# fperezgamonal/flownet2-tf

Hardware: AMD Instinct MI355X
Metric: forward pairs/sec at 512x384 (FlowNet2) (higher is better)
Workload: dtype f16x2 (split fp16 hi+lo operands, 3 fp16 MFMAs per product, fp32 accumulate); 1 GPU; FlowNet2 forward, batch=4 synthetic 512x384 pairs per GPU, seeded synthetic weights; pairs_per_gpu=4, parallelism=dp1 (no collective)

## Files before the change

flownet2-tf_amd/csrc/conv.hip:

```cpp
#include "conv_common.h"
#include <cstdlib>

namespace fn2 {

template <typename T, typename OutT, int TC, int WC, int WP>
__global__ void __launch_bounds__(256) conv_igemm_kernel(const ConvArgs p) {
  constexpr int CH = 16 / (int)sizeof(T);
  constexpr int BC = WC * TC * 16;
  constexpr int BP = WP * 64;
  constexpr int NT = 256;
  static_assert(WC * WP == 4, "4 waves per block");
  constexpr int NPR = BP / 64;
  constexpr int NWR = (BC * 4 + NT - 1) / NT;
  constexpr int WSWZ_BIT = (TC == 4) ? 5 : (TC == 2) ? 4 : 3;
  __shared__ uint4 lds[2][(BC + BP) * 4];

  const int tid = threadIdx.x, lane = tid & 63, wave = tid >> 6;
  const int wc = wave / WP, wp = wave % WP;
  const int cid = tid & 3;

  int pad_y = p.pad, pad_x = p.pad, oy_off = 0, ox_off = 0, osc = 1;
  const T* wgt = reinterpret_cast<const T*>(p.wgt);
  const int phase = blockIdx.z / p.splitk, split = blockIdx.z - phase * p.splitk;
  if (p.deconv) {
// ... 929 lines not shown
    const char* e_trim = getenv("FN2_TRIM_TAPS");
    if (!e_trim || atoi(e_trim) != 0)
      for (int ph = 0; ph < 2; ++ph) {
        const int ky0 = ph + d->pad + 2 * (ph ? a.ph_pad1 : a.ph_pad0);
        const int t = ky0 < 0 ? 0 : ky0 / 2 + 1;
        trim[ph] = t < T ? t : T;
      }
  }
  for (int ph = 0; ph < 2; ++ph) { a.kh_ph[ph] = trim[ph] > 0 ? trim[ph] : a.KH; a.kw_ph[ph] = trim[ph] > 0 ? trim[ph] : a.KW; }
  a.accum = d->accumulate ? 1 : 0;
  a.mask_y = d->act_grad_y; a.mask_c0 = d->act_grad_c0; a.mask_c1 = d->act_grad_c1;
  if (a.mask_y != nullptr) {
    FN2_REQUIRE(d->out.dtype == FN2_F32 || d->out.dtype == FN2_F16X2, "conv2d: act_grad_y needs an fp32 or split-fp16 output");
    FN2_REQUIRE(d->act == FN2_ACT_NONE && d->kind != 2, "conv2d: act_grad_y goes with a linear gradient layer (kinds 0, 1, 3)");
    FN2_REQUIRE(0 <= a.mask_c0 && a.mask_c0 < a.mask_c1 && a.mask_c1 <= d->out.c, "conv2d: act_grad channel range outside the output view");
    FN2_REQUIRE(!is_flow_head(d), "conv2d: act_grad_y is not available on the flow-head path");
  }
  if (a.accum) FN2_REQUIRE(d->out.dtype == FN2_F32 || d->out.dtype == FN2_F16X2,
                           "conv2d: accumulate needs an fp32 or split-fp16 output");
  const long M = (long)a.N * a.OH * a.OW;
  FN2_REQUIRE(M < (1L << 31), "conv2d: too many output pixels");
  a.M = (int)M;
  a.out_H = d->out.h; a.out_W = d->out.w; a.out_cs = d->out.cs; a.out_c0 = d->out.c0; a.Cout = d->out.c;
  FN2_REQUIRE(d->kpad >= a.KH * a.KW * d->cin_pad, "conv2d: kpad smaller than taps*cin_pad");
  a.ksteps = d->kpad / (4 * CH);
  a.cout_pad = d->cout_pad;
  a.act = d->act;
  a.out_scale = d->out_scale == 0.f ? 1.f : d->out_scale;
  a.vec_ok = (d->out.cs % 4 == 0) && (d->out.c0 % 4 == 0);
  a.splitk = 1; a.kper = a.ksteps; a.ws = nullptr; a.ws_cs = (a.Cout + 3) / 4 * 4;
  { const char* e = getenv("FN2_CONV_DBG"); a.dbg = e ? atoi(e) : 0; }
  a.in_bytes = 0;
  if (d->wgt_layout >= 1) {
    const long in_bytes = (long)d->in.n * d->in.h * d->in.w * d->in.cs * esz;
    FN2_REQUIRE(in_bytes < (1L << 31), "conv2d: input buffer >= 2 GiB is not addressable by the LDS-DMA kernel");
    FN2_REQUIRE((long)d->cout_pad * d->kpad * esz < (1L << 31), "conv2d: packed weight >= 2 GiB per phase");
    a.in_bytes = (int)in_bytes;
  }
  {
    const double A = (double)d->cout_pad * d->kpad * esz, B = (double)d->in.n * d->in.h * d->in.w * d->in.cs * esz;
    const long X = cdiv(M, 64), Y = cdiv(d->cout_pad, 128);
    const char* e = getenv("FN2_WMAJOR");
    const int mode = e ? atoi(e) : 2;
    a.wmajor = mode == 2 ? (A * (double)(X < 8 ? X : 8) + B > A + B * (double)(Y < 8 ? Y : 8)) : mode;
  }
  a.bp64 = wfrag ? 1 : wants_bp64(a, tile, phases, d->wgt_layout) ? 1 : 0;
  if ((a.dbg & 64) && d->wgt_layout == 1 && tile == 128 && !a.bp64) a.bp64 = 2;
  if (wfrag) {
    const char* e_wr = getenv("FN2_WREG_RING");
    const char* e_ring = getenv("FN2_RING_MAX");
    const int mode = e_wr ? atoi(e_wr) : 1;
    const long blocks = (long)cdiv(a.M, 64) * (a.cout_pad / 128) * phases;
    if (tile == 128 && (mode == 2 || (mode == 1 && blocks >= 384 && blocks <= (e_ring ? atoi(e_ring) : 512)))) a.wfrag = 2;
  }
  a.kg = 1;
  if (d->wgt_layout == 1 && tile == 128 && !(a.dbg & 32)) {
    const char* e_kg = getenv("FN2_KG");
    if (!e_kg || atoi(e_kg) != 0) {
      const char* e3 = getenv("FN2_KG3_MAX");
      const char* e2 = getenv("FN2_KG2_MAX");
      const long blocks = (long)cdiv(a.M, 64) * (a.cout_pad / 128) * phases;
      if (blocks <= (e3 ? atoi(e3) : 0)) { a.bp64 = 1; a.kg = 3; }
      else if (blocks <= (e2 ? atoi(e2) : 95)) { a.bp64 = 1; a.kg = 2; }
    }
  }
  if (d->wgt_layout == 1 && tile == 128 && !(a.dbg & 32) && d->in.dtype == FN2_F16X2) {
    const char* e_lo = getenv("FN2_DEEP_MIN");
    const char* e_hi = getenv("FN2_DEEP_MAX");
    const long blocks = (long)cdiv(a.M, 64) * (a.cout_pad / 128) * phases;
    const int lo = e_lo ? atoi(e_lo) : 0, hi = e_hi ? atoi(e_hi) : -1;
    if (blocks >= lo && blocks <= hi) { a.bp64 = 3; a.kg = 1; }
  }
  if (d->wgt_layout == 1 && tile == 128 && a.bp64 == 1 && a.kg == 1) {
    const char* e_ring = getenv("FN2_RING_MAX");
    const int ring_max = e_ring ? atoi(e_ring) : 512;
    const long blocks = (long)cdiv(a.M, 64) * (a.cout_pad / 128) * phases;
    if ((a.dbg & 256) || (blocks >= 384 && blocks <= ring_max)) a.bp64 = 2;
    const char* e_rs = getenv("FN2_RING_SPLIT");
    if (e_rs && blocks >= atoi(e_rs) && blocks < 384) a.bp64 = 2;
  }
  *tile_out = tile;
  *phases_out = phases;
  return FN2_OK;
}

static int preferred_split(const ConvArgs& a, int tile, int phases) {
  if (a.merged) return 1;
  const int bp = tile == 128 ? (a.bp64 ? 64 : 128) : (a.bp64 ? 128 : 256);
  const long blocks = (long)cdiv(a.M, bp) * (a.cout_pad / tile) * phases;
  const char* e_min = getenv("FN2_SPLIT_MINBLOCKS");
  if (blocks >= (e_min ? atoi(e_min) : 384)) return 1;
  if (a.bp64 == 3) {
    const char* e_sl = getenv("FN2_DEEP_SLOTS");
    int s = (int)((e_sl ? atoi(e_sl) : 256) / blocks);
    const int maxs = a.ksteps / 16;
    if (s > maxs) s = maxs;
    if (s > 16) s = 16;
    if (s < 2) return 1;
    const int kper = cdiv(a.ksteps, s);
    return cdiv(a.ksteps, kper);
  }
  if (a.kg > 1) {
    const char* e_nos = getenv("FN2_KG_NOSPLIT");
    if (blocks >= (e_nos ? atoi(e_nos) : 96)) return 1;
    const char* e_sl = getenv("FN2_KG_SLOTS");
    int s = (int)((e_sl ? atoi(e_sl) : 256) / blocks);
    const int maxs = a.ksteps / (12 * a.kg);
    if (s > maxs) s = maxs;
    if (s > 16) s = 16;
    if (s < 2) return 1;
    const int kper = cdiv(a.ksteps, s);
    return cdiv(a.ksteps, kper);
  }
  const char* e = getenv("FN2_SPLIT_SLOTS");
  const char* e_rsl = getenv("FN2_RING_SPLIT_SLOTS");
  const int slots = (tile == 128 && a.bp64 == 2) ? (e_rsl ? atoi(e_rsl) : 512) : e ? atoi(e) : 640;
  int s = (int)(slots / blocks);
  const int maxs = a.ksteps / 8;
  if (s > maxs) s = maxs;
  if (s > 16) s = 16;
  if (s < 2) return 1;
  const int kper = cdiv(a.ksteps, s);
  return cdiv(a.ksteps, kper);
}

static int64_t split_bytes(const ConvArgs& a, int s) {
  return (int64_t)s * a.N * a.out_H * a.out_W * a.ws_cs * (int64_t)sizeof(float);
}

}

extern "C" {

int64_t fn2_conv2d_workspace_bytes(const fn2_conv_desc* d) {
  ConvArgs a;
  int tile, phases;
  if (build_args(d, &a, &tile, &phases) != FN2_OK) return 0;
  if (is_flow_head(d)) return 0;
  const int s = preferred_split(a, tile, phases);
  return s > 1 ? split_bytes(a, s) : 0;
// ... 329 lines not shown
```

flownet2-tf_amd/csrc/conv2.hip:

```cpp
#include "conv_common.h"

#include <type_traits>
#include <algorithm>
#include <utility>

#ifndef FN2_X2_ORDER
#define FN2_X2_ORDER 0
#endif
#ifndef FN2_CONV_ABLATE
#define FN2_CONV_ABLATE 0
#endif
#ifndef FN2_SETPRIO
#define FN2_SETPRIO 1
#endif

namespace fn2 {

typedef __attribute__((address_space(3))) void* lptr_t;

constexpr unsigned kOobOffset = 0x80000000u;

typedef int v4i_t __attribute__((ext_vector_type(4)));
typedef unsigned u32x4_t __attribute__((ext_vector_type(4)));

// ... 345 lines not shown
      {
        const int ch = fh ^ fsw;
#pragma unroll
        for (int t = 0; t < TCN; ++t) fa[0][t] = A[t * 32 * 8 + ch];
#pragma unroll
        for (int t = 0; t < TPN; ++t) fb[0][t] = B[t * 32 * 8 + ch];
      }
#pragma unroll
      for (int ks = 0; ks < 4; ++ks) {
        const int cur = ks & 1, nxt = cur ^ 1;
        if (ks + 1 < 4) {
          const int ch = ((ks + 1) * 2 + fh) ^ fsw;
#pragma unroll
          for (int t = 0; t < TCN; ++t) fa[nxt][t] = A[t * 32 * 8 + ch];
#pragma unroll
          for (int t = 0; t < TPN; ++t) fb[nxt][t] = B[t * 32 * 8 + ch];
        }
        if constexpr (sizeof(T) == 2) {
#pragma unroll
          for (int tc = 0; tc < TCN; ++tc)
#pragma unroll
            for (int tp = 0; tp < TPN; ++tp)
              acc[tc][tp] = mfma_32x32x16<T>(fa[cur][tc], fb[cur][tp], acc[tc][tp]);
        } else {
#pragma unroll
          for (int j = 0; j < 4; ++j)
#pragma unroll
            for (int tc = 0; tc < TCN; ++tc)
#pragma unroll
              for (int tp = 0; tp < TPN; ++tp)
                acc[tc][tp] = __builtin_amdgcn_mfma_f32_32x32x2f32(__builtin_bit_cast(f32x4, fa[cur][tc])[j],
                                                                   __builtin_bit_cast(f32x4, fb[cur][tp])[j],
                                                                   acc[tc][tp], 0, 0, 0);
        }
      }
    }
#if FN2_SETPRIO
    __builtin_amdgcn_s_setprio(0);
#endif
  };

  auto compute_w = [&](const uint4* lds, const u32x4_t (&wf)[WREG ? 4 : 1]) {
    if constexpr (WREG) {
#if FN2_SETPRIO
      __builtin_amdgcn_s_setprio(1);
#endif
      const uint4* B = &lds[(BOFF + wp * TPN * 32 + fr) * 8];
#pragma unroll
      for (int q = 0; q < 2; ++q) {
        const int chh = (4 * q + 2 * fh) ^ fsw, chl = (4 * q + 2 * fh + 1) ^ fsw;
        uint4 bh[TPN], bl[TPN];
#pragma unroll
        for (int t = 0; t < TPN; ++t) { bh[t] = B[t * 32 * 8 + chh]; bl[t] = B[t * 32 * 8 + chl]; }
#pragma unroll
        for (int tp = 0; tp < TPN; ++tp) {
          const uint4 ah = __builtin_bit_cast(uint4, wf[2 * q]), al = __builtin_bit_cast(uint4, wf[2 * q + 1]);
          acc[0][tp] = mfma_32x32x16<f16_t>(al, bh[tp], acc[0][tp]);
          acc[0][tp] = mfma_32x32x16<f16_t>(ah, bl[tp], acc[0][tp]);
          acc[0][tp] = mfma_32x32x16<f16_t>(ah, bh[tp], acc[0][tp]);
        }
      }
#if FN2_SETPRIO
      __builtin_amdgcn_s_setprio(0);
#endif
    }
  };

  if constexpr (FEED) {
    const int nst3 = (kt1 - kt0 + 2) / 3 * 3;
    auto pix_stage = [&](uint4* lds) {
      [&]<int... I>(std::integer_sequence<int, I...>) {
        (issue_piece(std::integral_constant<int, NWI + I>{}, lds), ...);
      }(std::make_integer_sequence<int, NPI>{});
      advance();
    };
    if (feeder) {
      static_assert(NPI == 2, "vmcnt literal below");
      pix_stage(lds0);
      pix_stage(lds1);
      for (int s = 0; s < nst3; s += 3) {
        asm volatile("s_waitcnt vmcnt(2)\n\ts_barrier" ::: "memory"); pix_stage(lds2);
        asm volatile("s_waitcnt vmcnt(2)\n\ts_barrier" ::: "memory"); pix_stage(lds0);
        asm volatile("s_waitcnt vmcnt(2)\n\ts_barrier" ::: "memory"); pix_stage(lds1);
      }
      asm volatile("s_waitcnt vmcnt(0)" ::: "memory");
    } else {
      auto w_stage = [&](u32x4_t (&wf)[4]) { load_w(wf); advance(); };
      auto sync_c = [&](u32x4_t (&wf)[4]) {
        asm volatile("s_waitcnt vmcnt(4)\n\ts_barrier" : "+v"(wf[0]), "+v"(wf[1]), "+v"(wf[2]), "+v"(wf[3]) :: "memory");
      };
      w_stage(wfa);
      w_stage(wfb);
      for (int s = 0; s < nst3; s += 3) {
        sync_c(wfa); w_stage(wfc); compute_w(lds0, wfa);
        sync_c(wfb); w_stage(wfa); compute_w(lds1, wfb);
        sync_c(wfc); w_stage(wfb); compute_w(lds2, wfc);
      }
      asm volatile("s_waitcnt vmcnt(0)" : "+v"(wfa[0]), "+v"(wfa[1]), "+v"(wfa[2]), "+v"(wfa[3]), "+v"(wfb[0]), "+v"(wfb[1]),
                   "+v"(wfb[2]), "+v"(wfb[3]) :: "memory");
    }
  } else if constexpr (WREG && STAGES == 3) {
    static_assert(NPI + 4 == 6, "vmcnt literal below");
    auto ring_sync_w = [&](u32x4_t (&wf)[4]) {
      asm volatile("s_waitcnt vmcnt(6)\n\ts_barrier" : "+v"(wf[0]), "+v"(wf[1]), "+v"(wf[2]), "+v"(wf[3]) :: "memory");
    };
    issue_stage_w(lds0, wfa);
    issue_stage_w(lds1, wfb);
    const int nst3 = (kt1 - kt0 + 2) / 3 * 3;
    for (int s = 0; s < nst3; s += 3) {
      ring_sync_w(wfa); issue_stage_w(lds2, wfc); compute_w(lds0, wfa);
      ring_sync_w(wfb); issue_stage_w(lds0, wfa); compute_w(lds1, wfb);
      ring_sync_w(wfc); issue_stage_w(lds1, wfb); compute_w(lds2, wfc);
    }
    asm volatile("s_waitcnt vmcnt(0)" : "+v"(wfa[0]), "+v"(wfa[1]), "+v"(wfa[2]), "+v"(wfa[3]), "+v"(wfb[0]), "+v"(wfb[1]),
                 "+v"(wfb[2]), "+v"(wfb[3]) :: "memory");
  } else if constexpr (WREG) {
    issue_stage_w(lds0, wfa);
    wait_w(wfa);
    __syncthreads();
    const int nst2 = (kt1 - kt0 + 1) & ~1;
    for (int s = 0; s < nst2; s += 2) {
      issue_stage_w(lds1, wfb);
      compute_w(lds0, wfa);
      wait_w(wfb);
      __syncthreads();
      if (s + 2 < nst2) issue_stage_w(lds0, wfa);
      compute_w(lds1, wfb);
      wait_w(wfa);
      __syncthreads();
    }
  } else if constexpr (STAGES == 2) {
    issue_stage(lds0);
    asm volatile("s_waitcnt vmcnt(0)" ::: "memory");
    __syncthreads();
    const int nst2 = ((kt1 - (kt0 - grp) + KG - 1) / KG + 1) & ~1;
    for (int s = 0; s < nst2; s += 2) {
// ... 1119 lines not shown
#undef FN2_HALO
  return true;
}

ConvNameSink& conv_name_sink() {
  static thread_local ConvNameSink sink{nullptr, 0};
  return sink;
}

template <typename T, typename OutT>
static int launch2(const ConvArgs& a, int tile, int phases, hipStream_t s) {
  const int z = phases * a.splitk;
  const long blocks64 = (long)cdiv(a.M, 64) * (a.cout_pad / 128) * z;
  const char* e_m16 = getenv("FN2_M16_MIN");
  const bool m16 = is_x2<T>::value && !(a.dbg & 512) &&
                   ((a.dbg & 1024) || (e_m16 && tile == 128 && a.bp64 == 1 && a.kg == 1 && a.splitk == 1 &&
                                       blocks64 >= atoi(e_m16)));
#define FN2_LAUNCH2(GX, GY, THREADS, ...)                                                              \
  do {                                                                                                 \
    dim3 grid(GX, GY, z);                                                                              \
    if (conv_name_sink().buf)                                                                          \
      snprintf(conv_name_sink().buf, conv_name_sink().cap, "conv_igemm2_kernel<%s, %s, %s, %s>", type_name<T>(), \
               type_name<OutT>(), #__VA_ARGS__, m16 ? "true" : "false");                              \
    else if (m16) hipLaunchKernelGGL((conv_igemm2_kernel<T, OutT, __VA_ARGS__, is_x2<T>::value>), grid, dim3(THREADS), 0, s, a); \
    else hipLaunchKernelGGL((conv_igemm2_kernel<T, OutT, __VA_ARGS__, false>), grid, dim3(THREADS), 0, s, a);            \
  } while (0)
  if (a.wfrag) {
    if constexpr (is_x2<T>::value) {
      if (tile == 64) {
        dim3 grid(cdiv(a.M, 128), a.cout_pad / 64, z);
        if (conv_name_sink().buf)
          snprintf(conv_name_sink().buf, conv_name_sink().cap, "conv_igemm2_kernel<%s, %s, 2, 2, 1, 2, 2, 1, false, true, %s>",
                   type_name<T>(), type_name<OutT>(), a.splitk > 1 ? "true" : "false");
        else if (a.splitk > 1)
          hipLaunchKernelGGL((conv_igemm2_kernel<T, OutT, 2, 2, 1, 2, 2, 1, false, true, true>), grid, dim3(256), 0, s, a);
        else
          hipLaunchKernelGGL((conv_igemm2_kernel<T, OutT, 2, 2, 1, 2, 2, 1, false, true, false>), grid, dim3(256), 0, s, a);
      } else {
        dim3 grid(cdiv(a.M, 64), a.cout_pad / 128, z);
        const bool slab = a.splitk > 1;
        ConvArgs ah = a;
        if (a.fh_M > 0 && slab && !conv_name_sink().buf) {
          const char* e = getenv("FN2_FH_BLOCKS");
          const long per_z = (long)grid.x * grid.y;
          const long want = std::min<long>(a.fh_M, e ? atoi(e) : 1024);
          ah.fh_z0 = z;
          grid.z = z + (unsigned)std::max<long>(1, (want + per_z - 1) / per_z);
        } else {
          ah.fh_M = 0;
        }
        const ConvArgs& a = ah;
        const char* e_feed = getenv("FN2_WREG_FEED");
        const int feed = e_feed ? atoi(e_feed) : 1;
        if (conv_name_sink().buf)
          snprintf(conv_name_sink().buf, conv_name_sink().cap, "conv_igemm2_kernel<%s, %s, 4, 1, 1, 2, %d, 1, false, true, %s%s>",
                   type_name<T>(), type_name<OutT>(), a.wfrag == 2 ? 3 : 2, slab ? "true" : "false",
                   (a.wfrag == 2 && (slab ? feed >= 2 : feed >= 1)) ? ", false, true" : "");
        else if (a.wfrag == 2 && slab && feed >= 2)
          hipLaunchKernelGGL((conv_igemm2_kernel<T, OutT, 4, 1, 1, 2, 3, 1, false, true, true, false, true>), grid, dim3(512), 0, s, a);
        else if (a.wfrag == 2 && slab)
          hipLaunchKernelGGL((conv_igemm2_kernel<T, OutT, 4, 1, 1, 2, 3, 1, false, true, true>), grid, dim3(256), 0, s, a);
        else if (a.wfrag == 2 && feed >= 1)
          hipLaunchKernelGGL((conv_igemm2_kernel<T, OutT, 4, 1, 1, 2, 3, 1, false, true, false, false, true>), grid, dim3(512), 0, s, a);
        else if (a.wfrag == 2)
          hipLaunchKernelGGL((conv_igemm2_kernel<T, OutT, 4, 1, 1, 2, 3, 1, false, true, false>), grid, dim3(256), 0, s, a);
        else if (slab)
          hipLaunchKernelGGL((conv_igemm2_kernel<T, OutT, 4, 1, 1, 2, 2, 1, false, true, true>), grid, dim3(256), 0, s, a);
        else
          hipLaunchKernelGGL((conv_igemm2_kernel<T, OutT, 4, 1, 1, 2, 2, 1, false, true, false>), grid, dim3(256), 0, s, a);
      }
    } else {
      return fail(FN2_ERR_UNSUPPORTED, "conv fast path: fragment-order weights are split fp16 only");
    }
  } else if (tile == 128 && a.bp64 && a.kg == 3) FN2_LAUNCH2(cdiv(a.M, 64), a.cout_pad / 128, 768, 2, 2, 2, 1, 2, 3);
  else if (tile == 128 && a.bp64 && a.kg == 2) FN2_LAUNCH2(cdiv(a.M, 64), a.cout_pad / 128, 512, 2, 2, 2, 1, 2, 2);
  else if (tile == 128 && a.bp64 == 3) FN2_LAUNCH2(cdiv(a.M, 64), a.cout_pad / 128, 256, 2, 2, 2, 1, 6, 1);
  else if (tile == 128 && a.bp64 == 2) FN2_LAUNCH2(cdiv(a.M, 64), a.cout_pad / 128, 256, 2, 2, 2, 1, 3, 1);
  else if (tile == 128 && a.bp64) FN2_LAUNCH2(cdiv(a.M, 64), a.cout_pad / 128, 256, 2, 2, 2, 1, 2, 1);
  else if (tile == 128) FN2_LAUNCH2(cdiv(a.M, 128), a.cout_pad / 128, 256, 2, 2, 2, 2, 2, 1);
  else if (tile == 64 && a.bp64) FN2_LAUNCH2(cdiv(a.M, 128), a.cout_pad / 64, 256, 1, 4, 2, 1, 2, 1);
  else if (tile == 64) FN2_LAUNCH2(cdiv(a.M, 256), a.cout_pad / 64, 256, 1, 4, 2, 2, 2, 1);
  else if (a.bp64) FN2_LAUNCH2(cdiv(a.M, 128), a.cout_pad / 32, 256, 1, 4, 1, 1, 2, 1);
  else FN2_LAUNCH2(cdiv(a.M, 256), a.cout_pad / 32, 256, 1, 4, 1, 2, 2, 1);
#undef FN2_LAUNCH2
  return conv_launched("conv_igemm2");
}

int launch_head5_strip(const ConvArgs& a, int blocks, hipStream_t s) {
  if (a.ksteps != 3 && a.ksteps != 6) return fail(FN2_ERR_UNSUPPORTED, "flow_head5 strip form: %d channel lines (3 or 6)", a.ksteps);
  if (conv_name_sink().buf) FN2_CONV_NAME("head5_strip_kernel<%d>", a.ksteps / 3);
  else if (a.ksteps == 3) hipLaunchKernelGGL((head5_strip_kernel<1>), dim3(blocks), dim3(512), 0, s, a);
  else hipLaunchKernelGGL((head5_strip_kernel<2>), dim3(blocks), dim3(512), 0, s, a);
  return conv_launched("flow_head5_strip");
}

int launch_head5(const ConvArgs& a, int blocks, hipStream_t s) {
  if (conv_name_sink().buf)
    FN2_CONV_NAME("conv_igemm2_kernel<fn2::x2_t, float, 1, 4, 2, 2, 2, 1, false, false, false, true>");
  else
    hipLaunchKernelGGL((conv_igemm2_kernel<x2_t, float, 1, 4, 2, 2, 2, 1, false, false, false, true>), dim3(blocks, 1, 1), dim3(256), 0,
                       s, a);
  return conv_launched("flow_head5");
}

bool conv_fast_ok(int in_dtype, int cin_pad, int cout) {
  const int esz = dtype_size(in_dtype);
  return cout > 2 && (cin_pad * esz) % 128 == 0;
// ... 27 lines not shown
```

flownet2-tf_amd/src/_hip.py:

```python
import ctypes as C
import os

import numpy as np
import torch

_HERE = os.path.dirname(os.path.abspath(__file__))
LIB_PATH = os.path.join(os.path.dirname(_HERE), "lib", "libflownet2_hip.so")

FN2_F32, FN2_BF16, FN2_F16, FN2_F16X2 = 0, 1, 2, 3
ACT_NONE, ACT_LEAKY = 0, 1
OK = 0
ERR_INVALID_ARGUMENT, ERR_UNSUPPORTED, ERR_HIP = -1, -2, -3
MASK_F32, MASK_U8 = 0, 1
OPTIM_KINDS = {"sgd": 0, "momentum": 1, "adam": 2, "adamw": 3}
OPTIM_PARTIALS = 128


class Fn2Tensor(C.Structure):
    _fields_ = [("data", C.c_void_p), ("dtype", C.c_int32), ("n", C.c_int32), ("h", C.c_int32),
                ("w", C.c_int32), ("c", C.c_int32), ("cs", C.c_int32), ("c0", C.c_int32)]


class Fn2ConvPlan(C.Structure):
    _fields_ = [("layout", C.c_int32), ("cout_tile", C.c_int32), ("kstep_elems", C.c_int32),
                ("wgt_dtype", C.c_int32)]


class Fn2ConvDesc(C.Structure):
    _fields_ = [("inp", Fn2Tensor), ("out", Fn2Tensor), ("wgt", C.c_void_p), ("bias", C.c_void_p),
                ("kind", C.c_int32), ("kh", C.c_int32), ("kw", C.c_int32), ("stride", C.c_int32),
                ("pad", C.c_int32), ("act", C.c_int32), ("cin_pad", C.c_int32), ("cout_pad", C.c_int32),
                ("kpad", C.c_int32), ("wgt_layout", C.c_int32), ("accumulate", C.c_int32), ("out_scale", C.c_float), ("workspace", C.c_void_p), ("workspace_bytes", C.c_int64),
                ("act_grad_y", C.c_void_p), ("act_grad_c0", C.c_int32), ("act_grad_c1", C.c_int32),
                ("up_src", C.c_void_p), ("up_w", C.c_void_p), ("up_bias", C.c_void_p), ("up_c0", C.c_int32),
                ("head", C.c_void_p), ("raw_partials", C.c_int32)]


class Fn2BwdwDesc(C.Structure):
    _fields_ = [("x", Fn2Tensor), ("dy", Fn2Tensor), ("dw", C.c_void_p), ("kind", C.c_int32), ("kh", C.c_int32),
                ("kw", C.c_int32), ("stride", C.c_int32), ("pad", C.c_int32), ("cin_pad", C.c_int32),
                ("cout_pad", C.c_int32), ("kpad", C.c_int32), ("wgt_layout", C.c_int32), ("db", C.c_void_p)]


class Fn2HfemLevel(C.Structure):
    _fields_ = [("pred", C.c_void_p), ("label", C.c_void_p), ("epe", C.c_void_p), ("weight", C.c_void_p),
                ("npix", C.c_int64), ("k", C.c_int64), ("hard_weight", C.c_float)]


class Fn2PhotometricLevel(C.Structure):
    _fields_ = [("pred", C.c_void_p), ("img", C.c_void_p), ("mask", C.c_void_p), ("mask_sum", C.c_void_p),
                ("dpred", C.c_void_p), ("h", C.c_int32), ("w", C.c_int32), ("scale", C.c_float), ("weight", C.c_float)]


_i, _p, _f = C.c_int, C.c_void_p, C.c_float
_ip = C.POINTER(C.c_int)
_tp = C.POINTER(Fn2Tensor)

PROTOTYPES = {
    "fn2_last_error": (C.c_char_p, []),
    "fn2_version": (_i, []),
    "fn2_crc32c": (C.c_uint32, [_p, C.c_int64, C.c_uint32]),
    "fn2_device_info": (_i, [C.c_char_p, _i, _ip]),
    "fn2_correlation_out_shape": (_i, [_i] * 7 + [_ip] * 3),
    "fn2_correlation_f32": (_i, [_p, _p, _p] + [_i] * 9 + [_p]),
    "fn2_correlation_workspace_bytes": (C.c_int64, [_i] * 9),
    "fn2_correlation_f32_ws": (_i, [_p, _p, _p] + [_i] * 9 + [_p, C.c_int64, _p]),
    "fn2_correlation_f32_kernel_name": (_i, [_i] * 10 + [C.c_char_p, _i]),
    "fn2_correlation_grad_f32": (_i, [_p] * 5 + [_i] * 9 + [_p]),
    "fn2_correlation_grad_f32_kernel_name": (_i, [_i] * 9 + [C.c_char_p, _i]),
    "fn2_flow_warp_f32": (_i, [_p, _p, _p, _i, _i, _i, _i, _p]),
    "fn2_flow_warp_grad_f32": (_i, [_p] * 5 + [_i] * 4 + [_p]),
    "fn2_downsample_f32": (_i, [_p, _p] + [_i] * 6 + [_p]),
    "fn2_downsample_scaled_f32": (_i, [_p, _f, _p] + [_i] * 6 + [_p]),
    "fn2_fill_zero": (_i, [_p, C.c_int64, _p]),
    "fn2_add_f32": (_i, [_p, _p, C.c_int64, _p]),
    "fn2_slice_copy_f32": (_i, [_tp, _p, _p]),
    "fn2_resize_bilinear_f32": (_i, [_p, _p] + [_i] * 6 + [_f, _p]),
    "fn2_conv2d_plan": (_i, [_i, _i, _i, C.POINTER(Fn2ConvPlan)]),
    "fn2_conv2d_workspace_bytes": (C.c_int64, [C.POINTER(Fn2ConvDesc)]),
    "fn2_conv2d": (_i, [C.POINTER(Fn2ConvDesc), _p]),
    "fn2_conv2d_kernel_name": (_i, [C.POINTER(Fn2ConvDesc), C.c_char_p, _i]),
    "fn2_conv2d_splits": (_i, [C.POINTER(Fn2ConvDesc)]),
    "fn2_augment_f32": (_i, [_p, _p, _p, _p, _i, _i, _i, _i, _i, _i, _p]),
    "fn2_flow_augmentation_f32": (_i, [_p, _p, _p, _p, _i, _i, _i, _i, _i, _p]),
    "fn2_selflow_workspace_bytes": (C.c_int64, [_i, _i, _i]),
    "fn2_selflow_stats": (_i, [_p, _p, _p, _p, _p, C.c_int64, _i, _i, _i, _p]),
    "fn2_selflow_apply": (_i, [_p] * 15 + [C.c_int64, _i, _i, _i, _p]),
    "fn2_flow_head_gather": (_i, [_p, _i, _p, _p, _i, _i, _i, _p]),
# ... 138 lines not shown
```

flownet2-tf_amd/src/engine.py:

```python
import ctypes as C
import os
import types

import numpy as np
import torch

from . import _hip, netdefs, weights as W

_DT = {"f32": torch.float32, "bf16": torch.bfloat16, "f16": torch.float16, "f16x2": torch.float32}
_CODE = {"f32": _hip.FN2_F32, "bf16": _hip.FN2_BF16, "f16": _hip.FN2_F16, "f16x2": _hip.FN2_F16X2}


def _round_up(x, m):
    return (x + m - 1) // m * m


class BatchTooLarge(ValueError):

    def __init__(self, name, batch, nbytes, limit):
        self.fit = max(1, int(batch * (limit - 1) // nbytes))
        super().__init__("activation tensor %s of a batch of %d pairs is %d bytes (limit %d): at most %d pairs per engine"
                         % (name, batch, nbytes, limit, self.fit))


# ... 16 lines not shown
        self.act_code = _CODE[dtype]
        self.code_of = {}
        self.weights = weights
        if no_deconv_biases is None:
            no_deconv_biases = "FlowNetS/predict_flow6/biases" not in weights
        self.no_deconv_biases = bool(no_deconv_biases)
        self.consumed = set()
        self.ignored_variables = []
        self.ops = []
        self.kernel_of = []
        self.branch_of = []
        self._branch = 0
        self.desc_branch = []
        self.syncs = []
        self._lanes_on = bool(int(os.environ.get("FN2_BRANCHES", "1")))
        default_mask = 0b10011 if model == "FlowNet2" else (0b10101 if model == "FlowNetSD" else 0b10001)
        self._lane_mask = int(os.environ.get("FN2_LANE_MASK", str(default_mask)))
        self.keep = []
        self.bufs = {}
        self.layer_flops = []
        self.layer_bytes = []
        self.layer_io_bytes = []
        self.in_a = torch.zeros((self.N, self.H, self.W, 3), dtype=torch.float32, device=self.device)
        self.in_b = torch.zeros_like(self.in_a)
        self.uint8_inputs = bool(uint8_inputs)
        if self.uint8_inputs:
            self.in_a_u8 = torch.zeros((self.N, self.H, self.W, 3), dtype=torch.uint8, device=self.device)
            self.in_b_u8 = torch.zeros_like(self.in_a_u8)
            self._lut_div = torch.from_numpy((np.arange(256, dtype=np.float64) / 255.0).astype(np.float32)).to(self.device)
            self._lut_raw = torch.arange(256, dtype=torch.float32, device=self.device)
            self._lut = [self._lut_div.clone(), self._lut_div.clone()]
            self._lut_mode = [True, True]
            cnt = self.in_a_u8.numel()
            for src, lut, dst, nm in ((self.in_a_u8, self._lut[0], self.in_a, "a"), (self.in_b_u8, self._lut[1], self.in_b, "b")):
                self.kernel_of.append("u8_to_f32_lut_kernel")
                self.ops.append((f"input_{nm}/u8_to_f32", self.lib.fn2_u8_to_f32_lut,
                                 (_hip.ptr(src), _hip.ptr(lut), _hip.ptr(dst), cnt)))
                self.branch_of.append(0)
        self.interp_u8_inputs = bool(interp_u8_inputs)
        if self.interp_u8_inputs:
            if model != "FlowNetS_interp":
                raise ValueError("interp_u8_inputs belongs to FlowNetS_interp, not %s" % model)
            self.in_img_u8 = torch.zeros((self.N, self.H, self.W, 3), dtype=torch.uint8, device=self.device)
            self.in_mask_u8 = torch.zeros((self.N, self.H, self.W), dtype=torch.uint8, device=self.device)
            self.in_sparse = torch.zeros((self.N, self.H, self.W, 2), dtype=torch.float32, device=self.device)
            self.in_flags = torch.ones((self.N, 2), dtype=torch.uint8, device=self.device)
            self._lut_255 = torch.from_numpy((np.arange(256, dtype=np.float64) / 255.0).astype(np.float32)).to(self.device)
        self.graph = None
        self.conv_descs = []
        self.layers = []
        self.heads_as_gemm = heads_as_gemm
        self.plain_stems = bool(plain_stems)
        self.fragment_weights = bool(int(os.environ.get("FN2_WREG", "1"))) if fragment_weights is None else bool(fragment_weights)
        self.compose_heads = bool(heads_as_gemm) and dtype == "f16x2" and bool(int(os.environ.get("FN2_COMPOSE", "1")))
        self._head_t = {}
        self._defer_flow = False
        self._own_ws = set()
        self._pending_head = None
        self.outputs = self._build()
        assert self._pending_head is None
        self._check_variables(strict)
        self._alloc_workspace()
        self._resolve_kernel_names()

    def _buf(self, name, n, h, w, c, dtype=None, stem=False):
        line = 64 if self.act_code in (_hip.FN2_BF16, _hip.FN2_F16) else 32
        cs = (_round_up(c, line) if c > 32 else _round_up(c, 8)) if dtype is None else c
        if dtype is None and not stem and line == 32 and 8 < c <= 32:
            cs = 32

        td = self.tdtype if dtype is None else dtype
        nbytes = n * h * w * cs * torch.empty((), dtype=td).element_size()
        if nbytes >= self.MAX_TENSOR_BYTES:
            if self.N <= 1:
                raise ValueError("one %d x %d pair needs a %d-byte tensor (%s): above the %d-byte limit of the kernels"
                                 % (self.H, self.W, nbytes, name, self.MAX_TENSOR_BYTES))
            raise BatchTooLarge(name, self.N, nbytes, self.MAX_TENSOR_BYTES)
        t = torch.zeros((n, h, w, cs), dtype=td, device=self.device)
        assert name not in self.bufs, name
        self.bufs[name] = t
        self.code_of[t.data_ptr()] = self.act_code if dtype is None else _hip.FN2_F32
        return t

    def _code(self, buf):
        base = buf.untyped_storage().data_ptr()
        return self.code_of.get(buf.data_ptr(), self.code_of.get(base, _hip.dtype_code(buf)))

    def _v(self, buf, c=None, c0=0):
        return _hip.view(buf, c, c0, self._code(buf))

    def _w(self, key):
        if key not in self.weights:
            raise KeyError("the weights lack %r, a variable of the reference's %s graph" % (key, self.model))
        self.consumed.add(key)
        return self.weights[key]

    def _bias(self, scope, name, kind, cout):
        key = f"{scope}/{name}/biases"
        if not netdefs.has_bias(self.model, name, kind, self.no_deconv_biases):
            if key in self.weights:
                self.ignored_variables.append(key)
            return None
        b = np.asarray(self._w(key), np.float32).reshape(-1)
        if b.shape[0] != cout:
            raise ValueError("%s has %d entries, the layer has %d outputs" % (key, b.shape[0], cout))
        return W.to_device(b, torch.float32, self.device)
# ... 76 lines not shown
        d.accumulate = int(accumulate)
        d.out_scale = pk.out_scale
        self.keep += [d, bias]
        self.conv_descs.append(d)
        self.desc_branch.append(self._branch if lane is None else lane)
        return d

    def _packed_conv(self, src, dst, w_hwio, pack, kind=0, k=1, stride=1, pad=0, act=False, bias=None, cin_pad=None,
                     fragments=False):
        sbuf, sc0, sc = src
        dbuf, dc0, dc = dst
        pk = self._pack_weight(src, w_hwio, dc, pack, cin_pad)
        d = self._conv_desc(self._v(sbuf, sc, sc0), self._v(dbuf, dc, dc0), pk, kind, k, stride, pad, act, bias)
        pk.frag = bool(fragments and self.fragment_weights and pk.layout == 1 and pk.wgt_dtype == _hip.FN2_F16X2
                       and pk.tile >= int(os.environ.get("FN2_WREG_TILE_MIN", "128")) and self._wants_fragments(d))
        if pk.frag:
            pk.w = W.to_fragment_order(pk.w)
            d.wgt, d.wgt_layout = pk.w.data_ptr(), 2
        self.keep.append(pk.w)
        return d, pk

    @staticmethod
    def _layer_facts(pk):
        return dict(w=pk.w, cin_pad=pk.cin_pad, cout_pad=pk.cout_pad, kpad=pk.kpad, layout=pk.layout, tile=pk.tile,
                    kstep=pk.kstep)

    def _upflow_rec(self, scope, name, src_f32, dst):
        dbuf, dc0, dc = dst
        w = W.to_device(self._w(f"{scope}/{name}/weights"), torch.float32, self.device)
        b = self._bias(scope, name, "deconv", 2)
        v = self._v(dbuf, dc, dc0)
        self.keep += [w, b, v]
        self.layers.append(dict(scope=scope, name=name, kind="upflow", src=src_f32, dst=dst, w=w, b=b, view=v))
        return w, b, v

    def _conv(self, scope, spec, src, dst, up=None, up_after=None, defer_head=False):
        name, kind, k, stride, pad, cin, cout, act = spec
        sbuf, sc0, sc = src
        dbuf, dc0, dc = dst
        assert sc == cin and dc == cout, (scope, name, sc, cin, dc, cout)
        head_px = dbuf.shape[0] * dbuf.shape[1] * dbuf.shape[2]
        if (self.heads_as_gemm and kind == "conv" and cout == 2 and k == 3 and stride == 1 and pad == 1 and not act
                and dbuf.dtype == torch.float32 and head_px >= int(os.environ.get("FN2_HEAD_GEMM_MIN", "8192"))
                and self._head_gemm(scope, spec, src, dst, up)):
            return up is not None and bool(int(os.environ.get("FN2_FUSE_UPFLOW", "1")))
        in_code = self._code(sbuf)
        esz = 2 if in_code in (_hip.FN2_BF16, _hip.FN2_F16) else 4
        merged = (kind != "conv" and self.compose_heads and cout == 16 and in_code == _hip.FN2_F16X2
                  and sbuf.shape[2] % 128 == 0 and bool(int(os.environ.get("FN2_DECONV_MERGED", "1"))))
        pack, dkind = (W.pack_conv, 0) if kind == "conv" else (W.pack_deconv_merged, 5) if merged else (W.pack_deconv, 1)
        w_var = self._w(f"{scope}/{name}/weights")
        bias = self._bias(scope, name, kind, cout)
        d, pk = self._packed_conv(src, dst, w_var, pack, dkind, k, stride, pad, act, bias, fragments=True)
        if self._pending_head is not None and kind != "conv":
            hd = self._pending_head
            assert up_after is not None and hd.inp.data == d.inp.data and hd.inp.c0 == d.inp.c0, (scope, name)
            d.head = C.addressof(hd)
            self._pending_head = None
        self.layers.append(dict(scope=scope, name=name, kind=d.kind, k=k, stride=stride, pad=pad, cin=cin, cout=cout,
                                act=bool(act), src=src, dst=dst, desc=d, b=bias, frag=pk.frag, **self._layer_facts(pk)))
        if up_after is not None:
            assert kind != "conv" and (not merged or cout == 16)
            up_name, up_src, (ubuf, uc0, uc) = up_after
            assert ubuf is dbuf and uc == 2
            uw, ub, _ = self._upflow_rec(scope, up_name, up_src, up_after[2])
            d.up_src, d.up_w, d.up_bias, d.up_c0 = up_src.data_ptr(), uw.data_ptr(), (ub.data_ptr() if ub is not None else None), uc0
        if defer_head and kind == "conv" and cout == 2 and k == 3 and stride == 1 and pad == 1:
            assert self._pending_head is None
            self._pending_head = d
        else:
            self._op(f"{scope}/{name}", self.lib.fn2_conv2d, C.byref(d))
        n, oh, ow = dbuf.shape[0], dbuf.shape[1], dbuf.shape[2]
        taps = k * k if kind == "conv" else 4
        self.layer_flops.append((f"{scope}/{name}", 2.0 * n * oh * ow * taps * cin * cout))
        osz = 4 if dbuf.dtype == torch.float32 else 2
        self.layer_io_bytes.append((f"{scope}/{name}", float(sbuf.shape[0] * sbuf.shape[1] * sbuf.shape[2] * cin * esz
                                                            + n * oh * ow * cout * osz + k * k * cin * cout * esz)))

    def _head_slabs(self, d, head_t, t_cs):
        need = int(self.lib.fn2_conv2d_workspace_bytes(C.byref(d)))
        if need <= 0 or not int(os.environ.get("FN2_HEAD_SLABS", "1")):
            return _hip.ptr(head_t), t_cs, 1, 0, 1.0
        ws = torch.empty((need + 3) // 4, dtype=torch.float32, device=self.device)
        d.workspace, d.workspace_bytes, d.raw_partials = ws.data_ptr(), need, 1
        self.keep.append(ws)
        self._own_ws.add(C.addressof(d))
        splits = int(self.lib.fn2_conv2d_splits(C.byref(d)))
        if splits <= 1:
            d.raw_partials = 0
            return _hip.ptr(head_t), t_cs, 1, 0, 1.0
        ws_cs = (d.out.c + 3) // 4 * 4
        return ws.data_ptr(), ws_cs, splits, d.out.n * d.out.h * d.out.w * ws_cs, float(d.out_scale) or 1.0

    def _wants_fragments(self, d):
        need = int(self.lib.fn2_conv2d_workspace_bytes(C.byref(d)))
        d.workspace, d.workspace_bytes = (1, need) if need else (None, 0)
        buf = C.create_string_buffer(256)
        rc = self.lib.fn2_conv2d_kernel_name(C.byref(d), buf, 256)
        d.workspace, d.workspace_bytes = None, 0
        which = os.environ.get("FN2_WREG_KERNELS", "false>")
        return rc == 0 and buf.value.decode().startswith("conv_igemm2_kernel") and buf.value.decode().endswith(which)

    def _head_tail(self, scope, pf_name, partials, taps, ring, bias, pf, up):
        t_ptr, t_cs, nslab, slab, tscale = partials
        n, h, wd = pf.shape[0], pf.shape[1], pf.shape[2]
        label, uw, ub, uv = f"{scope}/{pf_name}/tail", None, None, None
        if up is not None:
            uw, ub, uv = self._upflow_rec(scope, up[0], pf, up[1])
            label += "+" + up[0]
        self._op(label, self.lib.fn2_flow_head_tail_slabs, t_ptr, t_cs, nslab, slab, C.c_float(tscale), taps,
                 _hip.ptr(bias) if bias is not None else None, _hip.ptr(pf), n, h, wd, ring,
                 _hip.ptr(uw) if uw is not None else None, _hip.ptr(ub) if ub is not None else None,
                 C.byref(uv) if uv is not None else None, kernel="flow_head_tail")

    def _gemm_head(self, scope, gemm_name, pf_name, src, pk, taps, ring, bias, pf, up):
        sbuf, sc0, sc = src
        width = 32 if taps == 3 else 64
        key = (self._branch, width)
        if key not in self._head_t:
            self._head_t[key] = torch.zeros((self.N * self.H * self.W, width), dtype=torch.float32, device=self.device)
        head_t = self._head_t[key]
        n, h, wd = pf.shape[0], pf.shape[1], pf.shape[2]
        d = self._conv_desc(self._v(sbuf, sc, sc0),
                            _hip.Fn2Tensor(head_t.data_ptr(), _hip.FN2_F32, n, h, wd, 2 * taps * taps, width, 0), pk)
        self.keep.append(pk.w)
        self._op(f"{scope}/{gemm_name}", self.lib.fn2_conv2d, C.byref(d))
        self._head_tail(scope, pf_name, self._head_slabs(d, head_t, width), taps, ring, bias, pf, up)

    def _head_gemm(self, scope, spec, src, dst, up=None):
        name, kind, k, stride, pad, cin, cout, act = spec
        sbuf, sc0, sc = src
        pf = dst[0]
        if not self._cin_run(self._code(sbuf), sbuf, sc0, sc, 18)[1]:
            return False
        w = np.asarray(self._w(f"{scope}/{name}/weights"), np.float32)
        w1 = np.ascontiguousarray(w.transpose(2, 0, 1, 3)).reshape(1, 1, cin, 18)
        pk = self._pack_weight(src, w1, 18, W.pack_conv, lds_only=True)
        bias = self._bias(scope, name, kind, cout)
        self.keep.append(bias)
        self._gemm_head(scope, name, name, src, pk, 3, 0, bias, pf,
                        up if int(os.environ.get("FN2_FUSE_UPFLOW", "1")) else None)
        n, h, wd = pf.shape[0], pf.shape[1], pf.shape[2]
        esz = 2 if self._code(sbuf) in (_hip.FN2_BF16, _hip.FN2_F16) else 4
        self.layer_flops.append((f"{scope}/{name}", 2.0 * n * h * wd * 9 * cin * 2))
        self.layer_io_bytes.append((f"{scope}/{name}", float(n * h * wd * (cin * esz + 2 * 4) + 18 * cin * esz)))
# ... 583 lines not shown
```

include/flownet2_hip.h:

```cpp
#ifndef FLOWNET2_HIP_H_
#define FLOWNET2_HIP_H_

#include <stddef.h>
#include <stdint.h>

#ifdef __cplusplus
extern "C" {
#endif

typedef enum {
  FN2_OK = 0,
  FN2_ERR_INVALID_ARGUMENT = -1,
  FN2_ERR_UNSUPPORTED = -2,
  FN2_ERR_HIP = -3
} fn2_status;

typedef enum { FN2_F32 = 0, FN2_BF16 = 1, FN2_F16 = 2, FN2_F16X2 = 3 } fn2_dtype;

typedef enum { FN2_ACT_NONE = 0, FN2_ACT_LEAKY = 1  } fn2_act;

typedef struct {
  void* data;
  int32_t dtype;
  int32_t n, h, w;
// ... 19 lines not shown
int fn2_correlation_f32_ws(const float* a, const float* b, float* out, int n, int h, int w, int c, int kernel_size,
                           int max_displacement, int stride_1, int stride_2, int pad, void* workspace,
                           int64_t workspace_bytes, void* stream);
int fn2_correlation_f32_kernel_name(int n, int h, int w, int c, int kernel_size, int max_displacement, int stride_1,
                                    int stride_2, int pad, int with_workspace, char* name, int cap);

int fn2_correlation_grad_f32(const float* grad_out, const float* a, const float* b, float* grad_a,
                             float* grad_b, int n, int h, int w, int c, int kernel_size,
                             int max_displacement, int stride_1, int stride_2, int pad, void* stream);
int fn2_correlation_grad_f32_kernel_name(int n, int h, int w, int c, int kernel_size, int max_displacement, int stride_1,
                                         int stride_2, int pad, char* name, int cap);

int fn2_flow_warp_f32(const float* image, const float* flow, float* out, int n, int h, int w, int c,
                      void* stream);

int fn2_flow_warp_grad_f32(const float* image, const float* flow, const float* grad_out,
                           float* image_grad, float* flow_grad, int n, int h, int w, int c,
                           void* stream);

int fn2_downsample_f32(const float* in, float* out, int n, int in_h, int in_w, int c, int out_h,
                       int out_w, void* stream);

int fn2_downsample_scaled_f32(const float* in, float in_scale, float* out, int n, int in_h, int in_w, int c, int out_h,
                              int out_w, void* stream);

int fn2_resize_bilinear_f32(const float* in, float* out, int n, int in_h, int in_w, int c, int out_h,
                            int out_w, float scale, void* stream);


typedef struct {
  fn2_tensor in;
  fn2_tensor out;
  const void* wgt;
  const float* bias;
  int32_t kind;
  int32_t kh, kw, stride, pad;
  int32_t act;
  int32_t cin_pad;
  int32_t cout_pad;
  int32_t kpad;
  int32_t wgt_layout;
  int32_t accumulate;
  float out_scale;
  void* workspace;
  int64_t workspace_bytes;
  const void* act_grad_y;
  int32_t act_grad_c0, act_grad_c1;
  const float* up_src;
  const float* up_w;
  const float* up_bias;
  int32_t up_c0;
  const void* head;
  int32_t raw_partials;
} fn2_conv_desc;

typedef struct {
  int32_t layout, cout_tile, kstep_elems, wgt_dtype;
} fn2_conv_plan;
int fn2_conv2d_plan(int in_dtype, int cin_pad, int cout, fn2_conv_plan* plan);
int64_t fn2_conv2d_workspace_bytes(const fn2_conv_desc* d);
int fn2_conv2d(const fn2_conv_desc* d, void* stream);
int fn2_conv2d_kernel_name(const fn2_conv_desc* desc, char* name, int cap);
int fn2_conv2d_splits(const fn2_conv_desc* desc);

int fn2_flow_head_gather(const float* t, int t_cs, const float* bias, float* out, int n, int h, int w, void* stream);
int fn2_flow_head_tail(const float* t, int t_cs, int taps, const float* bias, float* pf, int n, int h, int w, int ring,
                       const float* up_w, const float* up_bias, const fn2_tensor* up_out, void* stream);
int fn2_flow_head_tail_slabs(const float* t, int t_cs, int nslab, int64_t slab_stride, float scale, int taps, const float* bias,
                             float* pf, int n, int h, int w, int ring, const float* up_w, const float* up_bias,
                             const fn2_tensor* up_out, void* stream);
int fn2_flow_head5(const fn2_tensor* x, const void* wgt, int cin_pad, int kpad, float out_scale, const float* bias, float* pf,
                   int ring, const float* ring_w, const float* ring_b, void* stream);
int fn2_flow_head5_kernel_name(const fn2_tensor* x, const void* wgt, int cin_pad, int kpad, float out_scale, const float* bias,
                               float* pf, int ring, const float* ring_w, const float* ring_b, char* name, int cap);
int fn2_flow_head_ring(const fn2_tensor* x, const float* wc, const float* bc, float* pf, void* stream);
int fn2_upsample_flow(const float* in, const float* w, const float* bias, const fn2_tensor* out, int n, int h, int wd,
                      void* stream);

int fn2_u8_to_f32_lut(const unsigned char* src, const float* lut256, float* dst, long count, void* stream);

int fn2_pack_pair(const float* a, const float* b, const fn2_tensor* out, int pad, void* stream);
int fn2_pack_interp_u8(const unsigned char* img, const unsigned char* mask, const float* sparse, const float* lut256,
                       const unsigned char* flags, const fn2_tensor* out, int pad, void* stream);
int fn2_pack_image(const float* img, int n_img, const fn2_tensor* out, int n0, int pad, void* stream);
int fn2_pack_image_s2d(const float* img, int n_img, int h, int w, const fn2_tensor* out, int n0, int pad, void* stream);

int fn2_correlation_fused(const fn2_tensor* a, const fn2_tensor* b, const fn2_tensor* out,
                          int max_displacement, int stride_2, int act, void* stream);
int fn2_correlation_fused_kernel_name(const fn2_tensor* a, const fn2_tensor* b, const fn2_tensor* out,
                                      int max_displacement, int stride_2, char* name, int cap);

int fn2_stack_input(const float* a, const float* b, const float* flow, const fn2_tensor* out, int pad,
                    void* stream);

int fn2_fusion_input(const float* a, const float* b, const float* flow_sd, const float* flow_css,
                     const fn2_tensor* out, int pad, void* stream);
int fn2_stack_input_pf(const float* a, const float* b, const float* pf, int pf_h, int pf_w, float scale, float* flow_out,
                       const fn2_tensor* out, int pad, void* stream);
int fn2_fusion_input_pf(const float* a, const float* b, const float* pf_sd, float scale_sd, float* flow_sd_out,
                        const float* pf_css, float scale_css, float* flow_css_out, int pf_h, int pf_w,
                        const fn2_tensor* out, int pad, void* stream);


int fn2_epe_loss_grad(const float* pred, const float* label, float* dpred, float* loss_accum, int n, int h, int w,
                      float weight, float grad_mult, void* stream);
int fn2_epe_loss_grad_weighted(const float* pred, const float* label, const float* pixel_weight, float* dpred,
// ... 111 lines not shown
```

Measured before the change: 1135 pairs/s.

## Add 128x96 pixel-tile register-weight ring variant for mid-sized convs

Adds a new wfrag=3 path that launches the register-fragment weight kernel with a 96-pixel tile (three pixel pieces per stage, 512 threads). It is selected for eligible convs inside FlowNetS sub-networks when the 96-pixel block count is at most 256, and it disables split-K for those convs. The aim is better wave fill and weight reuse on layers with few blocks. It also reorders the three MFMA passes so that independent tiles interleave when TPN>=3, which relaxes accumulator dependency chains. The risks are lower occupancy, higher register pressure, and losing split-K parallelism.

```diff
diff --git a/flownet2-tf_amd/csrc/conv.hip b/flownet2-tf_amd/csrc/conv.hip
--- a/flownet2-tf_amd/csrc/conv.hip
+++ b/flownet2-tf_amd/csrc/conv.hip
@@ -1005,6 +1005,14 @@
     const int mode = e_wr ? atoi(e_wr) : 1;
     const long blocks = (long)cdiv(a.M, 64) * (a.cout_pad / 128) * phases;
     if (tile == 128 && (mode == 2 || (mode == 1 && blocks >= 384 && blocks <= (e_ring ? atoi(e_ring) : 512)))) a.wfrag = 2;
+    const char* e_force = getenv("FN2_PX96_FORCE");
+    const bool force = e_force && atoi(e_force) != 0;
+    const long blocks96 = (long)cdiv(a.M, 96) * (a.cout_pad / 128) * phases;
+    const char* e_feed = getenv("FN2_WREG_FEED");
+    if (d->px96 && tile == 128 && (!e_feed || atoi(e_feed) >= 1) && (d->kind == 0 || d->kind == 1) && !a.accum && a.mask_y == nullptr &&
+        (d->out.dtype == FN2_F16X2 || d->out.dtype == FN2_F32) && !is_flow_head(d) &&
+        (force || (mode == 1 && a.wfrag == 2 && blocks96 <= 256)))
+      a.wfrag = 3;
   }
   a.kg = 1;
   if (d->wgt_layout == 1 && tile == 128 && !(a.dbg & 32)) {
@@ -1039,6 +1047,7 @@
 
 static int preferred_split(const ConvArgs& a, int tile, int phases) {
   if (a.merged) return 1;
+  if (a.wfrag == 3) return 1;
   const int bp = tile == 128 ? (a.bp64 ? 64 : 128) : (a.bp64 ? 128 : 256);
   const long blocks = (long)cdiv(a.M, bp) * (a.cout_pad / tile) * phases;
   const char* e_min = getenv("FN2_SPLIT_MINBLOCKS");
diff --git a/flownet2-tf_amd/csrc/conv2.hip b/flownet2-tf_amd/csrc/conv2.hip
--- a/flownet2-tf_amd/csrc/conv2.hip
+++ b/flownet2-tf_amd/csrc/conv2.hip
@@ -421,12 +421,21 @@
         uint4 bh[TPN], bl[TPN];
 #pragma unroll
         for (int t = 0; t < TPN; ++t) { bh[t] = B[t * 32 * 8 + chh]; bl[t] = B[t * 32 * 8 + chl]; }
-#pragma unroll
-        for (int tp = 0; tp < TPN; ++tp) {
-          const uint4 ah = __builtin_bit_cast(uint4, wf[2 * q]), al = __builtin_bit_cast(uint4, wf[2 * q + 1]);
-          acc[0][tp] = mfma_32x32x16<f16_t>(al, bh[tp], acc[0][tp]);
-          acc[0][tp] = mfma_32x32x16<f16_t>(ah, bl[tp], acc[0][tp]);
-          acc[0][tp] = mfma_32x32x16<f16_t>(ah, bh[tp], acc[0][tp]);
+        const uint4 ah = __builtin_bit_cast(uint4, wf[2 * q]), al = __builtin_bit_cast(uint4, wf[2 * q + 1]);
+        if constexpr (TPN >= 3) {
+#pragma unroll
+          for (int tp = 0; tp < TPN; ++tp) acc[0][tp] = mfma_32x32x16<f16_t>(al, bh[tp], acc[0][tp]);
+#pragma unroll
+          for (int tp = 0; tp < TPN; ++tp) acc[0][tp] = mfma_32x32x16<f16_t>(ah, bl[tp], acc[0][tp]);
+#pragma unroll
+          for (int tp = 0; tp < TPN; ++tp) acc[0][tp] = mfma_32x32x16<f16_t>(ah, bh[tp], acc[0][tp]);
+        } else {
+#pragma unroll
+          for (int tp = 0; tp < TPN; ++tp) {
+            acc[0][tp] = mfma_32x32x16<f16_t>(al, bh[tp], acc[0][tp]);
+            acc[0][tp] = mfma_32x32x16<f16_t>(ah, bl[tp], acc[0][tp]);
+            acc[0][tp] = mfma_32x32x16<f16_t>(ah, bh[tp], acc[0][tp]);
+          }
         }
       }
 #if FN2_SETPRIO
@@ -444,13 +453,17 @@
       advance();
     };
     if (feeder) {
-      static_assert(NPI == 2, "vmcnt literal below");
+      static_assert(NPI == 2 || NPI == 3, "vmcnt literal below");
+      auto feed_sync = [] {
+        if constexpr (NPI == 2) asm volatile("s_waitcnt vmcnt(2)\n\ts_barrier" ::: "memory");
+        else asm volatile("s_waitcnt vmcnt(3)\n\ts_barrier" ::: "memory");
+      };
       pix_stage(lds0);
       pix_stage(lds1);
       for (int s = 0; s < nst3; s += 3) {
-        asm volatile("s_waitcnt vmcnt(2)\n\ts_barrier" ::: "memory"); pix_stage(lds2);
-        asm volatile("s_waitcnt vmcnt(2)\n\ts_barrier" ::: "memory"); pix_stage(lds0);
-        asm volatile("s_waitcnt vmcnt(2)\n\ts_barrier" ::: "memory"); pix_stage(lds1);
+        feed_sync(); pix_stage(lds2);
+        feed_sync(); pix_stage(lds0);
+        feed_sync(); pix_stage(lds1);
       }
       asm volatile("s_waitcnt vmcnt(0)" ::: "memory");
     } else {
@@ -1676,7 +1689,15 @@
         const ConvArgs& a = ah;
         const char* e_feed = getenv("FN2_WREG_FEED");
         const int feed = e_feed ? atoi(e_feed) : 1;
-        if (conv_name_sink().buf)
+        if (a.wfrag == 3) {
+          if (slab) return fail(FN2_ERR_UNSUPPORTED, "conv fast path: the 128 x 96 ring takes no K split");
+          grid.x = cdiv(a.M, 96);
+          if (conv_name_sink().buf)
+            snprintf(conv_name_sink().buf, conv_name_sink().cap, "conv_igemm2_kernel<%s, %s, 4, 1, 1, 3, 3, 1, false, true, false, false, true>",
+                     type_name<T>(), type_name<OutT>());
+          else
+            hipLaunchKernelGGL((conv_igemm2_kernel<T, OutT, 4, 1, 1, 3, 3, 1, false, true, false, false, true>), grid, dim3(512), 0, s, a);
+        } else if (conv_name_sink().buf)
           snprintf(conv_name_sink().buf, conv_name_sink().cap, "conv_igemm2_kernel<%s, %s, 4, 1, 1, 2, %d, 1, false, true, %s%s>",
                    type_name<T>(), type_name<OutT>(), a.wfrag == 2 ? 3 : 2, slab ? "true" : "false",
                    (a.wfrag == 2 && (slab ? feed >= 2 : feed >= 1)) ? ", false, true" : "");
diff --git a/flownet2-tf_amd/src/_hip.py b/flownet2-tf_amd/src/_hip.py
--- a/flownet2-tf_amd/src/_hip.py
+++ b/flownet2-tf_amd/src/_hip.py
@@ -33,7 +33,7 @@
                 ("kpad", C.c_int32), ("wgt_layout", C.c_int32), ("accumulate", C.c_int32), ("out_scale", C.c_float), ("workspace", C.c_void_p), ("workspace_bytes", C.c_int64),
                 ("act_grad_y", C.c_void_p), ("act_grad_c0", C.c_int32), ("act_grad_c1", C.c_int32),
                 ("up_src", C.c_void_p), ("up_w", C.c_void_p), ("up_bias", C.c_void_p), ("up_c0", C.c_int32),
-                ("head", C.c_void_p), ("raw_partials", C.c_int32)]
+                ("head", C.c_void_p), ("raw_partials", C.c_int32), ("px96", C.c_int32)]
 
 
 class Fn2BwdwDesc(C.Structure):
diff --git a/flownet2-tf_amd/src/engine.py b/flownet2-tf_amd/src/engine.py
--- a/flownet2-tf_amd/src/engine.py
+++ b/flownet2-tf_amd/src/engine.py
@@ -92,6 +92,7 @@
         self.heads_as_gemm = heads_as_gemm
         self.plain_stems = bool(plain_stems)
         self.fragment_weights = bool(int(os.environ.get("FN2_WREG", "1"))) if fragment_weights is None else bool(fragment_weights)
+        self.px96 = int(os.environ.get("FN2_WREG_PX96", "3")) if heads_as_gemm else 0
         self.compose_heads = bool(heads_as_gemm) and dtype == "f16x2" and bool(int(os.environ.get("FN2_COMPOSE", "1")))
         self._head_t = {}
         self._defer_flow = False
@@ -274,6 +275,8 @@
         w_var = self._w(f"{scope}/{name}/weights")
         bias = self._bias(scope, name, kind, cout)
         d, pk = self._packed_conv(src, dst, w_var, pack, dkind, k, stride, pad, act, bias, fragments=True)
+        if pk.frag:
+            d.px96 = int(self._wants_px96(scope))
         if self._pending_head is not None and kind != "conv":
             hd = self._pending_head
             assert up_after is not None and hd.inp.data == d.inp.data and hd.inp.c0 == d.inp.c0, (scope, name)
@@ -313,6 +316,13 @@
             return _hip.ptr(head_t), t_cs, 1, 0, 1.0
         ws_cs = (d.out.c + 3) // 4 * 4
         return ws.data_ptr(), ws_cs, splits, d.out.n * d.out.h * d.out.w * ws_cs, float(d.out_scale) or 1.0
+
+    def _wants_px96(self, scope):
+        if self.px96 == 2:
+            return self._branch == 0
+        if self.px96 == 3:
+            return self.model != "FlowNet2" or scope.endswith("/FlowNetS")
+        return self.px96 == 1
 
     def _wants_fragments(self, d):
         need = int(self.lib.fn2_conv2d_workspace_bytes(C.byref(d)))
diff --git a/include/flownet2_hip.h b/include/flownet2_hip.h
--- a/include/flownet2_hip.h
+++ b/include/flownet2_hip.h
@@ -95,6 +95,7 @@
   int32_t up_c0;
   const void* head;
   int32_t raw_partials;
+  int32_t px96;
 } fn2_conv_desc;
 
 typedef struct {
```

New measurement: 1139 pairs/s (median of 6 runs). About the same (+0.4%).
